# databendlabs/databend

Measured on AMD Instinct MI355X. Metric: rows/s TPC-H Q1 hash-agg, higher is better.
Workload: dtype i64/i128 decimal

## Files before the change

### databend_amd/csrc/gbk_api.h

```cpp

extern "C" {

int32_t dbhip_group_hash(const dbhip_col* cols, int32_t ncols, int64_t n, uint64_t* out_hashes,
                         void* stream) {
  DBHIP_REQUIRE(cols && ncols >= 1 && ncols <= GB_MAX_KEYS, "dbhip_group_hash: bad column list");
  if (n == 0) return DBHIP_OK;
  DBHIP_REQUIRE(out_hashes, "dbhip_group_hash: NULL out");
  HashCols hc;
  hc.n = ncols;
  for (int k = 0; k < ncols; ++k) {
    if (!key_type_ok(cols[k].type)) {
      set_error("dbhip_group_hash: unsupported type %d", cols[k].type);
      return DBHIP_ERR_INVALID;
    }
    hc.c[k] = to_gbcol(cols[k]);
  }
  hipStream_t s = resolve_stream(stream);
  unsigned long long* bad = (unsigned long long*)scratch(8, 2, s);
  if (!bad) return DBHIP_ERR_HIP;
  DBHIP_CHECK(hipMemsetAsync(bad, 0, 8, s));
  hipLaunchKernelGGL(group_hash_kernel, dim3(grid_for(ceil_div(n, 4), 256, 1024)), dim3(256), 0, s, hc, n, out_hashes, bad);
  DBHIP_LAUNCH_CHECK();
  return DBHIP_OK;
}
// ... 287 lines not shown
  g->rows_seen = 0;
}
static int32_t ensure_xcur(dbhip_groupby* g);
constexpr int GB_CTRL_XSTATUS = 12;
static int32_t blocks_queued(dbhip_groupby* g, const uint64_t* blocks, int32_t n_blocks, int64_t max_rows, int32_t skip, bool replace,
                             const char* who, hipStream_t s) {
  const int W = g->L.W;
  const int64_t stride = (max_rows + 1) * W;
  const int64_t ub = (int64_t)(n_blocks - (skip >= 0 && skip < n_blocks ? 1 : 0)) * max_rows;
  if (ub == 0) return DBHIP_OK;
  int32_t rc;
  if ((rc = ensure_xcur(g))) return rc;
  if ((rc = ensure((void**)&g->rows_in, &g->rows_in_cap, (size_t)ub * W * 8))) return rc;
  if ((rc = ensure((void**)&g->gid, &g->gid_cap, (size_t)ub * 4))) return rc;
  if ((rc = ensure((void**)&g->retry, &g->retry_cap, (size_t)ub * 4))) return rc;
  uint64_t* host = pinned_words(0);
  if (!host) return DBHIP_ERR_HIP;
  uint64_t* xst = g->ctrl + GB_CTRL_XSTATUS;
  if (replace)
    hipLaunchKernelGGL(gb_reset_unless_off_kernel, dim3(grid_for(g->cap, 256, 256)), dim3(256), 0, s, blocks, stride, n_blocks, max_rows, g->slot_hash, g->cap, g->ctrl);
  hipLaunchKernelGGL(gb_compact_blocks_kernel, dim3(n_blocks), dim3(256), 0, s, blocks, stride, W, skip, g->rows_in, xst, n_blocks, max_rows, replace ? 1 : 0);
  DBHIP_LAUNCH_CHECK();
  if ((rc = merge_rows_unpinned(g, g->rows_in, ub, s, xst, xst + 1, 2))) return rc;
  DBHIP_CHECK(hipMemcpyAsync(host, g->ctrl, (GB_CTRL_XSTATUS + 3) * sizeof(uint64_t), hipMemcpyDeviceToHost, s));
  DBHIP_CHECK(hipStreamSynchronize(s));
  if (host[GB_CTRL_XSTATUS + 1]) {
    set_error("%s: block %d overflowed max_rows=%lld (exchange the rows with dbhip_groupby_flush_partitioned / flush_serialized + "
              "merge_serialized instead)", who, (int)host[GB_CTRL_XSTATUS + 2] - 1, (long long)max_rows);
    return DBHIP_ERR_CAPACITY;
  }
  if (replace) reset_host_state(g);
  g->count_host = (int64_t)host[0];
  if (host[3] & 2) {
    set_error("groupby: a string key longer than 12 bytes was met; keep the CPU operator for this block");
    return DBHIP_ERR_UNSUPPORTED;
  }
  if (host[1]) {
    set_error("groupby: collision chain filled the table during retry; create the table with a larger capacity");
    return DBHIP_ERR_CAPACITY;
  }
  return host[GB_CTRL_XSTATUS] ? pin_string_states(g, s) : DBHIP_OK;
}

int32_t dbhip_groupby_merge_blocks(dbhip_groupby* g, const void* blocks_dev, int32_t n_blocks, int64_t max_rows,
                                   int32_t skip_block, void* stream) {
  GB_DRAIN(g, resolve_stream(stream));
  DBHIP_REQUIRE(g && blocks_dev && n_blocks >= 1 && n_blocks <= 4096 && max_rows >= 1, "dbhip_groupby_merge_blocks: bad argument");
  if (int32_t rl = refuse_long_strings(g, "dbhip_groupby_merge_blocks")) return rl;
// ... 329 lines not shown
```

### databend_amd/csrc/gbk_merge_lds.h

```cpp

namespace {

int32_t ensure(void** p, size_t* cap, size_t bytes) {
  if (*cap >= bytes) return DBHIP_OK;
  if (*p) {
    int32_t rc = dbhip_free(*p);
    if (rc) return rc;
    *p = nullptr; *cap = 0;
  }
  size_t want = bytes + (bytes >> 3) + 256;
  int32_t rc = dbhip_alloc(want, p);
  if (rc) { *p = nullptr; return rc; }
  *cap = want;
  return DBHIP_OK;
}

int32_t alloc_table(dbhip_groupby* g, int64_t cap, hipStream_t s) {
  uint64_t* nh = nullptr;
  uint64_t* nr = nullptr;
  int32_t rc = dbhip_alloc((size_t)cap * 8, (void**)&nh);
  if (rc == DBHIP_OK) rc = dbhip_alloc((size_t)cap * g->L.W * 8, (void**)&nr);
  hipError_t e = rc == DBHIP_OK ? hipMemsetAsync(nh, 0, (size_t)cap * 8, s) : hipSuccess;
  if (rc != DBHIP_OK || e != hipSuccess) {
    if (nh) (void)dbhip_free(nh);
// ... 131 lines not shown
  DBHIP_CHECK(hipMemsetAsync(&g->ctrl[8], 0, 8, s));
  hipLaunchKernelGGL(gb_pin_strings_kernel, dim3(grid), dim3(256), 0, s, g->L, g->slot_hash, g->rows, g->cap, (uint64_t)g->arena,
                     (uint64_t)g->arena + g->arena_cap, 4, na, (int64_t)0, g->ctrl, acc);
  DBHIP_LAUNCH_CHECK();
  DBHIP_CHECK(hipStreamSynchronize(s));
  trace("groupby: string arena compacted, %llu bytes in use -> %llu live (capacity %zu -> %zu)",
        (unsigned long long)two[1], (unsigned long long)two[0], g->arena_cap, want);
  (void)dbhip_free(g->arena);
  g->arena = na;
  g->arena_cap = want;
  return DBHIP_OK;
}
int32_t reserve_arena_for_chunk(dbhip_groupby* g, hipStream_t s) {
  uint64_t lb = 0;
  DBHIP_CHECK(hipMemcpyAsync(&lb, &g->ctrl[9], 8, hipMemcpyDeviceToHost, s));
  DBHIP_CHECK(hipStreamSynchronize(s));
  if (lb == 0) return DBHIP_OK;
  g->has_long = 1;
  return reserve_arena(g, lb, s);
}
bool layout_has_strings(const GbLayout& L) { return L.str_w1_mask != 0; }
bool layout_has_wide_minmax(const GbLayout& L);

int32_t merge_rows_unpinned(dbhip_groupby* g, const uint64_t* rows_in, int64_t n, hipStream_t s, const uint64_t* n_dev, const uint64_t* abort_dev,
                            int deferred = 0);
int32_t merge_rows(dbhip_groupby* g, const uint64_t* rows_in, int64_t n, hipStream_t s,
                   const uint64_t* n_dev = nullptr, const uint64_t* abort_dev = nullptr) {
  int32_t rc = merge_rows_unpinned(g, rows_in, n, s, n_dev, abort_dev);
  if (rc == DBHIP_OK && n > 0) rc = pin_string_states(g, s);
  return rc;
}
int32_t merge_rows_unpinned(dbhip_groupby* g, const uint64_t* rows_in, int64_t n, hipStream_t s,
                            const uint64_t* n_dev, const uint64_t* abort_dev, int deferred) {
  if (n == 0) return DBHIP_OK;
  if (n > 0xFFFFFFF0LL) {
    set_error("groupby: more than 2^32 rows in one call");
    return DBHIP_ERR_INVALID;
  }
  int32_t rc;
  if ((rc = ensure((void**)&g->gid, &g->gid_cap, (size_t)n * 4))) return rc;
  if ((rc = ensure((void**)&g->retry, &g->retry_cap, (size_t)n * 4))) return rc;
  const int grid = grid_for(n, 256);
  uint64_t* host_ctrl = pinned_words(0);
  if (!host_ctrl) return DBHIP_ERR_HIP;
  const uint64_t* cur_rows = rows_in;
  int64_t cur_n = n;
  const DevCount dc{n_dev, abort_dev};
  if ((deferred || (g->count_host + n) * 135 <= g->cap * 100) && n <= 256) {
    hipLaunchKernelGGL(gb_merge_small_kernel, dim3(1), dim3(256), 0, s, g->L, cur_rows, cur_n, g->slot_hash, g->rows, g->cap, g->hash_mask, g->gid,
                       g->retry, g->ctrl, dc, g->arena);
    DBHIP_LAUNCH_CHECK();
    if (deferred) return DBHIP_OK;
    DBHIP_CHECK(hipMemcpyAsync(host_ctrl, g->ctrl, 5 * sizeof(uint64_t), hipMemcpyDeviceToHost, s));
    DBHIP_CHECK(hipStreamSynchronize(s));
    g->count_host = (int64_t)host_ctrl[0];
    if (host_ctrl[3] & 2) {
      set_error("groupby: a string key longer than 12 bytes was met; keep the CPU operator for this block");
      return DBHIP_ERR_UNSUPPORTED;
    }
    if (host_ctrl[1]) {
      set_error("groupby: collision chain filled the table during retry; create the table with a larger capacity");
      return DBHIP_ERR_CAPACITY;
    }
    return DBHIP_OK;
  }
  if (deferred || (g->count_host + n) * 135 <= g->cap * 100) {
    DBHIP_CHECK(hipMemsetAsync(&g->ctrl[1], 0, 16, s));
    hipLaunchKernelGGL(gb_probe_kernel, dim3(grid), dim3(256), 0, s, g->L, cur_rows, cur_n, g->slot_hash, g->rows, g->cap,
                       g->hash_mask, g->gid, g->ctrl, dc, g->arena);
    if (deferred == 1 || (!deferred && g->count_host > 0 && g->count_host <= 32 && n <= 65536) || n <= 2048 || layout_has_wide_minmax(g->L))
      hipLaunchKernelGGL(gb_accum_lowcard_kernel, dim3(deferred == 1 && grid > 16 ? 16 : grid), dim3(256), 0, s, g->L, cur_rows, cur_n, g->rows, g->gid, g->retry,
// ... 323 lines not shown
```

### databend_amd/csrc/gbk_rows.h

```cpp

namespace {

struct HashCols {
  GbCol c[GB_MAX_KEYS];
  int n;
};

__global__ __launch_bounds__(256) void group_hash_kernel(HashCols hc, int64_t n, uint64_t* out,
                                                         unsigned long long* bad) {
  constexpr int U = 4;
  const int64_t T = (int64_t)gridDim.x * blockDim.x;
  const int64_t t = (int64_t)blockIdx.x * blockDim.x + threadIdx.x;
  for (int64_t base = 0; base < n; base += U * T) {
    int64_t row[U];
    bool in[U];
    uint64_t h[U];
#pragma unroll
    for (int u = 0; u < U; ++u) {
      row[u] = base + u * T + t;
      in[u] = row[u] < n;
      if (!in[u]) row[u] = n - 1;
      h[u] = 0;
    }
    for (int k = 0; k < hc.n; ++k) {
// ... 315 lines not shown

__device__ __forceinline__ uint64_t wave_min_u64(uint64_t v) {
#pragma unroll
  for (int off = 32; off >= 1; off >>= 1) {
    uint64_t o = __shfl_xor(v, off, 64);
    v = o < v ? o : v;
  }
  return v;
}
__device__ __forceinline__ uint64_t wave_max_u64(uint64_t v) {
#pragma unroll
  for (int off = 32; off >= 1; off >>= 1) {
    uint64_t o = __shfl_xor(v, off, 64);
    v = o > v ? o : v;
  }
  return v;
}
__device__ __forceinline__ double wave_sum_f64(double v) {
#pragma unroll
  for (int off = 32; off >= 1; off >>= 1) v += __shfl_xor(v, off, 64);
  return v;
}

__device__ __forceinline__ void gb_accum_lowcard_body(const GbLayout& L, const uint64_t* rows_in,
                                                      int64_t n, uint64_t* rows,
                                                      const uint32_t* gid, uint32_t* retry,
                                                      uint64_t* ctrl, const uint8_t* arena) {
  const int64_t n_pad = (n + 63) & ~63LL;
  for (int64_t i = (int64_t)blockIdx.x * blockDim.x + threadIdx.x; i < n_pad;
       i += (int64_t)gridDim.x * blockDim.x) {
    bool active = i < n;
    const uint64_t* r = rows_in + (active ? i : 0) * L.W;
    uint32_t pos = active ? gid[i] : GB_INVALID_SLOT;
    if (active) {
      const uint64_t* d = rows + (uint64_t)pos * L.W;
      if (!keys_equal(L, r, d, arena)) {
        unsigned long long k = atomicAdd((unsigned long long*)&ctrl[2], 1ULL);
        retry[k] = (uint32_t)i;
        active = false;
      }
    }
    uint64_t todo = __ballot(active);
    while (todo) {
      int leader = __ffsll((long long)todo) - 1;
      uint32_t lpos = __shfl(pos, leader, 64);
      bool mine = active && pos == lpos;
// ... 95 lines not shown
  }
}
__global__ void gb_retry_kernel(GbLayout L, const uint64_t* rows_in, uint64_t* slot_hash, uint64_t* rows,
                                int64_t cap, uint64_t hash_mask, const uint32_t* gid,
                                const uint32_t* retry, uint64_t* ctrl, uint8_t* arena) {
  if (threadIdx.x != 0 || blockIdx.x != 0) return;
  gb_retry_body(L, rows_in, slot_hash, rows, cap, hash_mask, gid, retry, ctrl, arena);
}

__global__ __launch_bounds__(256) void gb_merge_small_kernel(GbLayout L, const uint64_t* rows_in, int64_t n, uint64_t* slot_hash, uint64_t* rows,
                                                             int64_t cap, uint64_t hash_mask, uint32_t* gid, uint32_t* retry, uint64_t* ctrl,
                                                             DevCount dc, uint8_t* arena) {
  n = dev_rows(dc, n);
  if (threadIdx.x < 2) ctrl[1 + threadIdx.x] = 0;
  __threadfence();
  __syncthreads();
  gb_probe_body(L, rows_in, n, slot_hash, rows, cap, hash_mask, gid, ctrl, arena);
  __threadfence();
  __syncthreads();
  gb_accum_lowcard_body(L, rows_in, n, rows, gid, retry, ctrl, arena);
  __threadfence();
  __syncthreads();
  if (threadIdx.x == 0) gb_retry_body(L, rows_in, slot_hash, rows, cap, hash_mask, gid, retry, ctrl, arena);
}

__global__ __launch_bounds__(256) void gb_rehash_kernel(GbLayout L, const uint64_t* old_hash,
                                                        const uint64_t* old_rows, int64_t old_cap,
                                                        uint64_t* new_hash, uint64_t* new_rows,
                                                        int64_t new_cap, uint64_t hash_mask) {
  const uint64_t cmask = (uint64_t)new_cap - 1;
  for (int64_t s = (int64_t)blockIdx.x * blockDim.x + threadIdx.x; s < old_cap;
       s += (int64_t)gridDim.x * blockDim.x) {
    uint64_t hw = old_hash[s];
    if (hw == 0) continue;
    const uint64_t* r = old_rows + s * L.W;
    uint64_t pos = home_slot(probe_word(r[L.hash_word], hash_mask), new_cap);
    while (true) {
      unsigned long long old = atomicCAS((unsigned long long*)&new_hash[pos], 0ULL, (unsigned long long)hw);
      if (old == 0) break;
      pos = (pos + 1) & cmask;
    }
    uint64_t* d = new_rows + pos * L.W;
    for (int k = 0; k < L.W; ++k) d[k] = r[k];
  }
}

// ... 493 lines not shown
```

### databend_amd/csrc/k_fagg.hip

```cpp
#include "fagg_device.h"
#include "runtime.h"

#include <dirent.h>
#include <dlfcn.h>
#include <errno.h>
#include <sys/stat.h>
#include <fcntl.h>
#include <signal.h>
#include <spawn.h>
#include <sys/wait.h>
#include <unistd.h>

#include <atomic>
#include <chrono>
#include <deque>
#include <map>
#include <mutex>
#include <string>

#include <stdlib.h>
#include <string.h>
#include <time.h>

using namespace dbhip;

int32_t dbhip_groupby_merge_rows_dev_internal(dbhip_groupby* g, const uint64_t* rows, int64_t n_max, const uint64_t* n_dev,
                                              const uint64_t* abort_dev, hipStream_t s);
int32_t dbhip_groupby_merge_rows_internal(dbhip_groupby* g, const uint64_t* rows, int64_t n, hipStream_t s);
int64_t dbhip_groupby_capacity_internal(dbhip_groupby* g);
int32_t dbhip_groupby_reserve_merge_internal(dbhip_groupby* g, int64_t n);
int64_t dbhip_groupby_count_internal(dbhip_groupby* g);
const GbLayout* dbhip_groupby_layout_internal(dbhip_groupby* g);
int32_t dbhip_groupby_merge_rows_deferred_internal(dbhip_groupby* g, const uint64_t* rows, int64_t n_max, const uint64_t* n_dev,
                                                   const uint64_t* abort_dev, hipStream_t s);
int32_t dbhip_groupby_ensure_room_internal(dbhip_groupby* g, int64_t extra, hipStream_t s);
uint64_t* dbhip_groupby_ctrl_internal(dbhip_groupby* g);
void dbhip_groupby_set_count_internal(dbhip_groupby* g, int64_t count);
void** dbhip_groupby_pipe_slot_internal(dbhip_groupby* g);

namespace {

#include "build/jit_embed.inc"

struct JitOut {
  std::string s;
  void num(long long v) { s += std::to_string(v); s += ","; }
  void u64(uint64_t v) { char b[40]; snprintf(b, sizeof(b), "0x%llxULL,", (unsigned long long)v); s += b; }
  void null() { s += "nullptr,"; }
  void open() { s += "{"; }
  void close() { s += "},"; }
};

void jit_ins(JitOut& o, const ExIns& I) {
// ... 879 lines not shown
    pp->bound = true; pp->stream = s;
    return fa_pipe_enqueue(g, pp, P, s);
  }
  FaArgs A;
  memset(&A, 0, sizeof(A));
  bool general = false, may_raise = false;
  int nwords = 0;
  int32_t rc = fa_build_args(L, keys, prog, A, &general, &nwords, &may_raise);
  if (rc) return rc;
  A.filter_bits = filter_bitmap; A.filter_off = filter_bit_offset; A.n = n;
  A.has_filter = filter_bitmap != nullptr;
  const size_t lds = (size_t)(A.P.n_slots > 6 ? A.P.n_slots : 6) * FA_ROWS * 256 * 8;
  if (lds > 60 * 1024) {
    set_error("dbhip_groupby_add_block_program: %d live LDS slots exceed the register file; split the expression", A.P.n_slots);
    return DBHIP_ERR_UNSUPPORTED;
  }
  const int64_t nchunks = ceil_div(n, 64 * FA_ROWS);
  const int grid = (int)(ceil_div(nchunks, 4) < 512 ? ceil_div(nchunks, 4) : 512);
  if (FaPipe* pp = (FaPipe*)*dbhip_groupby_pipe_slot_internal(g); pp && !t_prepare_only) {
    int64_t committed = 0;
    if ((rc = fa_pipe_checkpoint(g, pp, &committed, true))) return rc;
  }
  const size_t rows_bytes = (size_t)grid * FA_MAX_SLOTS * L.W * 8;
  uint8_t* ws = (uint8_t*)scratch(rows_bytes + 64, 6, s);
  if (!ws) return DBHIP_ERR_HIP;
  uint64_t* ctrl = (uint64_t*)ws;
  A.ctrl = ctrl;
  A.partial_rows = (uint64_t*)(ws + 64);
  A.P.err_words = nullptr;
  A.P.err_count = (unsigned long long*)&ctrl[2];
  uint64_t* host_ctrl = pinned_words(1);
  if (!host_ctrl) return DBHIP_ERR_HIP;
  host_ctrl[0] = host_ctrl[1] = host_ctrl[2] = 0;
  const int64_t n_max = (int64_t)grid * FA_MAX_SLOTS;
  const bool chained = (dbhip_groupby_count_internal(g) + n_max) * 135 <= dbhip_groupby_capacity_internal(g) * 100;
  if ((rc = dbhip_groupby_reserve_merge_internal(g, n_max))) return rc;
  if (t_prepare_only) {
    (void)jit_kernel(A, dbhip_groupby_count_internal(g) > 4 ? 8 : 4, general, nwords, JIT_COMPILE);
    if (FaPipe* pq = (FaPipe*)*dbhip_groupby_pipe_slot_internal(g); pq && pq->on)
      (void)jit_kernel(A, dbhip_groupby_count_internal(g) > 4 ? 8 : 4, general, nwords, JIT_COMPILE, nullptr, true);
    return DBHIP_OK;
  }
  for (int variant = dbhip_groupby_count_internal(g) > 4 ? 1 : 0; variant < 2; ++variant) {
    DBHIP_CHECK(hipMemsetAsync(ctrl, 0, 64, s));
    kernel_timer_start(s);
    if ((rc = fa_launch(A, variant == 0 ? 4 : 8, general, nwords, grid, lds, s))) return rc;
    kernel_timer_stop(s);
    DBHIP_LAUNCH_CHECK();
    DBHIP_CHECK(hipMemcpyAsync(host_ctrl, ctrl, 24, hipMemcpyDeviceToHost, s));
    if (chained && !may_raise) {
      rc = dbhip_groupby_merge_rows_dev_internal(g, A.partial_rows, n_max, &ctrl[0], &ctrl[1], s);
      if (rc) return rc;
      if (!(host_ctrl[1] & 3)) return DBHIP_OK;
    } else {
      DBHIP_CHECK(hipStreamSynchronize(s));
    }
    if (!(host_ctrl[1] & 1)) break;
  }
  if (host_ctrl[1] & 2) {
    set_error("dbhip_groupby_add_block_program: a group key string is longer than 12 bytes");
    return DBHIP_ERR_UNSUPPORTED;
  }
  if (host_ctrl[1] & 1) {
    set_error("dbhip_groupby_add_block_program: more than %d distinct groups inside one workgroup; use the operator-at-a-time path", FA_MAX_SLOTS);
    return DBHIP_ERR_CAPACITY;
  }
  if (host_ctrl[2]) {
    set_error("dbhip_groupby_add_block_program: %llu row error(s) in the fused maps (Decimal overflow / divided by zero); "
              "evaluate the maps with dbhip_expr_eval to get the rows", (unsigned long long)host_ctrl[2]);
    return DBHIP_ERR_ROW_ERRORS;
  }
  return dbhip_groupby_merge_rows_internal(g, A.partial_rows, (int64_t)host_ctrl[0], s);
}

int32_t dbhip_groupby_set_pipelined(dbhip_groupby* g, int32_t on, void* stream) {
  DBHIP_REQUIRE(g, "dbhip_groupby_set_pipelined: NULL argument");
  void** slot = dbhip_groupby_pipe_slot_internal(g);
// ... 203 lines not shown
```

### databend_amd/csrc/k_groupby.hip

```cpp
#include <mutex>
#include "gb_device.h"
#include "runtime.h"

#include <math.h>
#include <stdlib.h>
#include <string.h>

#include <new>
#include <vector>

using namespace dbhip;

#define GB_INVALID_SLOT 0xFFFFFFFFu

struct dbhip_groupby {
  int64_t hint_groups;
  GbLayout L;
  int64_t cap;
  uint64_t* slot_hash;
  uint64_t* rows;
  uint64_t* ctrl;
  uint64_t hash_mask;
  int64_t count_host;
  uint64_t* rows_in; size_t rows_in_cap;
// ... 10 lines not shown
  int part_direct;
  int part_adapt;
  int part_validate, part_validated;
  int64_t rows_seen;
  uint32_t* part_meta; size_t part_meta_cap;
  uint32_t* spill_idx; size_t spill_idx_cap;
  uint64_t* spill_rows; size_t spill_rows_cap;
  uint8_t* arena; size_t arena_cap;
  int has_long;
  uint64_t* xcur;
  int xcur_dirty;
  int fagg_disabled;
  int gbc_off;
  int gbc_active;
  int gbc_lcap;
  int gbc_nodirect;
  int gbc_part_lcap_max;
  uint32_t gbc_part_cap;
  uint64_t* gbc_spill; size_t gbc_spill_cap;
  uint64_t arena_pinned, arena_live;
  int gbc_skip;
  uint32_t* gbc_split; size_t gbc_split_cap;
  void* fa_pipe;
};

int32_t dbhip_fagg_pipe_drain_internal(dbhip_groupby* g, void* pipe, hipStream_t s);
void dbhip_fagg_pipe_destroy_internal(void* pipe);
int32_t dbhip_fagg_pipe_reset_internal(void* pipe, hipStream_t s);
struct GbCols;
int32_t dbhip_fagg_pipe_add_columns_internal(dbhip_groupby* g, void* pipe, const GbCols& C, int64_t n, hipStream_t s);
#define GB_DRAIN(g, s)                                                                   \
  do {                                                                                   \
    if ((g) && (g)->fa_pipe) {                                                           \
      const int32_t _rc = dbhip_fagg_pipe_drain_internal((g), (g)->fa_pipe, (s));        \
      if (_rc) return _rc;                                                               \
    }                                                                                    \
  } while (0)

#include "gbk_rows.h"
int32_t dbhip_groupby_build_layout_internal(const int32_t* key_types, const uint8_t* key_nullable, int nkeys, const dbhip_agg_desc* aggs,
                                            int naggs, GbLayout* L) {
  return build_layout(key_types, key_nullable, nkeys, aggs, naggs, L);
}
#include "gbk_merge_lds.h"
int32_t dbhip_fagg_add_columns_internal(dbhip_groupby* g, const GbCols& C, int64_t row0, int64_t n, bool may_compile, hipStream_t s);
bool dbhip_fagg_last_refusal_is_pending_internal();
#include "gbk_partitioned.h"

int32_t dbhip_groupby_merge_rows_internal(dbhip_groupby* g, const uint64_t* rows, int64_t n, hipStream_t s) {
  return merge_rows(g, rows, n, s);
}
int32_t dbhip_groupby_merge_rows_dev_internal(dbhip_groupby* g, const uint64_t* rows, int64_t n_max, const uint64_t* n_dev,
                                              const uint64_t* abort_dev, hipStream_t s) {
  return merge_rows(g, rows, n_max, s, n_dev, abort_dev);
}
int32_t dbhip_groupby_reserve_merge_internal(dbhip_groupby* g, int64_t n) {
  int32_t rc;
  if ((rc = ensure((void**)&g->gid, &g->gid_cap, (size_t)n * 4))) return rc;
  return ensure((void**)&g->retry, &g->retry_cap, (size_t)n * 4);
}
int32_t dbhip_groupby_merge_rows_deferred_internal(dbhip_groupby* g, const uint64_t* rows, int64_t n_max, const uint64_t* n_dev,
                                                   const uint64_t* abort_dev, hipStream_t s) {
  return merge_rows_unpinned(g, rows, n_max, s, n_dev, abort_dev, 1);
}
int32_t dbhip_groupby_ensure_room_internal(dbhip_groupby* g, int64_t extra, hipStream_t s) {
  uint64_t cnt = 0;
  DBHIP_CHECK(hipMemcpyAsync(&cnt, &g->ctrl[0], 8, hipMemcpyDeviceToHost, s));
  DBHIP_CHECK(hipStreamSynchronize(s));
  g->count_host = (int64_t)cnt;
  while ((g->count_host + extra) * 135 > g->cap * 100) {
    const int32_t rc = grow(g, s);
    if (rc) return rc;
  }
  return DBHIP_OK;
}
uint64_t* dbhip_groupby_ctrl_internal(dbhip_groupby* g) { return g->ctrl; }
void dbhip_groupby_set_count_internal(dbhip_groupby* g, int64_t count) { g->count_host = count; }
void** dbhip_groupby_pipe_slot_internal(dbhip_groupby* g) { return &g->fa_pipe; }
// ... 6 lines not shown
```

### databend_amd/csrc/k_q1.hip

```cpp
#include "gb_device.h"
#include "runtime.h"

#include <stdlib.h>
#include <string.h>

using namespace dbhip;

int32_t dbhip_groupby_merge_rows_internal(dbhip_groupby* g, const uint64_t* rows, int64_t n, hipStream_t s);
int32_t dbhip_groupby_merge_rows_dev_internal(dbhip_groupby* g, const uint64_t* rows, int64_t n_max, const uint64_t* n_dev,
                                              const uint64_t* abort_dev, hipStream_t s);
int64_t dbhip_groupby_capacity_internal(dbhip_groupby* g);
int64_t dbhip_groupby_count_internal(dbhip_groupby* g);
const GbLayout* dbhip_groupby_layout_internal(dbhip_groupby* g);

namespace {

constexpr int MAX_SLOTS = 8;
constexpr int Q1_W = 15;

struct alignas(16) U4 {
  uint32_t x, y, z, w;
};
struct alignas(16) L2 {
  int64_t a, b;
};
struct alignas(8) I2 {
  int32_t a, b;
};

typedef uint32_t q1_u32x4 __attribute__((ext_vector_type(4)));
typedef uint32_t q1_u32x2 __attribute__((ext_vector_type(2)));
__device__ __forceinline__ U4 ld_u4(const U4* p) { return __builtin_bit_cast(U4, __builtin_nontemporal_load((const q1_u32x4*)p)); }
__device__ __forceinline__ L2 ld_l2(const int64_t* p) { return __builtin_bit_cast(L2, __builtin_nontemporal_load((const q1_u32x4*)p)); }
__device__ __forceinline__ I2 ld_i2(const int32_t* p) { return __builtin_bit_cast(I2, __builtin_nontemporal_load((const q1_u32x2*)p)); }

// ... 264 lines not shown

int32_t dbhip_q1_fused(dbhip_groupby* g, const int64_t* l_quantity, const int64_t* l_extendedprice,
                       const int64_t* l_discount, const int64_t* l_tax, const void* l_returnflag_views,
                       const void* l_linestatus_views, const int32_t* l_shipdate, int32_t shipdate_cutoff,
                       int64_t n, void* stream) {
  DBHIP_REQUIRE(g, "dbhip_q1_fused: NULL table");
  const GbLayout* L = dbhip_groupby_layout_internal(g);
  bool layout_ok = L->nkeys == 2 && L->naggs == 6 && L->W == Q1_W && L->key_type[0] == DBHIP_T_STRING &&
                   L->key_type[1] == DBHIP_T_STRING && L->agg_off[0] == 5 && L->agg_off[2] == 7 &&
                   L->agg_off[5] == 14 && L->agg_words[2] == 3 && L->agg_words[3] == 3;
  DBHIP_REQUIRE(layout_ok, "dbhip_q1_fused: table was not created by dbhip_q1_create_groupby");
  if (n == 0) return DBHIP_OK;
  DBHIP_REQUIRE(l_quantity && l_extendedprice && l_discount && l_tax && l_returnflag_views &&
                    l_linestatus_views && l_shipdate,
                "dbhip_q1_fused: NULL column");
  uintptr_t al = (uintptr_t)l_quantity | (uintptr_t)l_extendedprice | (uintptr_t)l_discount |
                 (uintptr_t)l_tax | (uintptr_t)l_returnflag_views | (uintptr_t)l_linestatus_views;
  DBHIP_REQUIRE((al & 15) == 0 && ((uintptr_t)l_shipdate & 7) == 0,
                "dbhip_q1_fused: columns must be 16-byte aligned (shipdate 8-byte)");
  hipStream_t s = resolve_stream(stream);
  const int64_t ntiles = ceil_div(n, 128);
  const int grid = (int)(ceil_div(ntiles, 4) < 512 ? ceil_div(ntiles, 4) : 512);
  size_t rows_bytes = (size_t)grid * MAX_SLOTS * Q1_W * 8;
  uint8_t* ws = (uint8_t*)scratch(rows_bytes + 64, 4, s);
  if (!ws) return DBHIP_ERR_HIP;
  uint64_t* ctrl = (uint64_t*)ws;
  uint64_t* partial = (uint64_t*)(ws + 64);
  Q1Args A;
  A.qty = l_quantity; A.price = l_extendedprice; A.disc = l_discount; A.tax = l_tax;
  A.rf = (const U4*)l_returnflag_views; A.ls = (const U4*)l_linestatus_views;
  A.shipdate = l_shipdate; A.cutoff = shipdate_cutoff; A.n = n;
  A.partial_rows = partial; A.ctrl = ctrl;
  uint64_t* host_ctrl = pinned_words(1);
  if (!host_ctrl) return DBHIP_ERR_HIP;
  host_ctrl[0] = host_ctrl[1] = 0;
  const int64_t n_max4 = (int64_t)grid * 4, n_max8 = (int64_t)grid * MAX_SLOTS;
  const bool chained = (dbhip_groupby_count_internal(g) + n_max8) * 135 <= dbhip_groupby_capacity_internal(g) * 100;
  for (int variant = 0; variant < 2; ++variant) {
    DBHIP_CHECK(hipMemsetAsync(ctrl, 0, 64, s));
    kernel_timer_start(s);
    if (variant == 0) hipLaunchKernelGGL(q1_fused_kernel, dim3(grid), dim3(256), 0, s, A);
    else hipLaunchKernelGGL(q1_fused_kernel_8slots, dim3(grid), dim3(256), 0, s, A);
    kernel_timer_stop(s);
    DBHIP_LAUNCH_CHECK();
    DBHIP_CHECK(hipMemcpyAsync(host_ctrl, ctrl, 16, hipMemcpyDeviceToHost, s));
    if (chained) {
      int32_t rc = dbhip_groupby_merge_rows_dev_internal(g, partial, variant == 0 ? n_max4 : n_max8, &ctrl[0], &ctrl[1], s);
      if (rc) return rc;
      if (!(host_ctrl[1] & 3)) return DBHIP_OK;
    } else {
      DBHIP_CHECK(hipStreamSynchronize(s));
    }
    if (!(host_ctrl[1] & 1)) break;
  }
  if (host_ctrl[1] & 2) {
    set_error("dbhip_q1_fused: a group key string is longer than 12 bytes; use the operator-at-a-time path");
    return DBHIP_ERR_UNSUPPORTED;
  }
  if (host_ctrl[1] & 1) {
    set_error("dbhip_q1_fused: more than %d distinct groups inside one workgroup; use the operator-at-a-time path", MAX_SLOTS);
    return DBHIP_ERR_CAPACITY;
  }
  return dbhip_groupby_merge_rows_internal(g, partial, (int64_t)host_ctrl[0], s);
}

}
```

### databend_amd/csrc/runtime.h

```cpp
#pragma once
#include <hip/hip_runtime.h>
#include <stdint.h>
#include <stdio.h>
#include <stdlib.h>

#include "../../include/dbhip.h"

namespace dbhip {

void set_error(const char* fmt, ...);
hipStream_t resolve_stream(void* stream);
int32_t hip_fail(hipError_t e, const char* what);

void* scratch(size_t bytes, int slot, hipStream_t stream);
void release_stream_scratch(hipStream_t stream);

bool cancel_requested(hipStream_t stream);

uint64_t* pinned_words(int slot);

void kernel_timer_start(hipStream_t s);
void kernel_timer_stop(hipStream_t s);


void trace(const char* fmt, ...) __attribute__((format(printf, 1, 2)));

inline int64_t ceil_div(int64_t a, int64_t b) { return (a + b - 1) / b; }

inline int grid_for(int64_t n_items_per_thread_units, int block, int cap = 2048) {
  int64_t need = ceil_div(n_items_per_thread_units, block);
  if (need < 1) need = 1;
  if (need > cap) need = cap;
  return (int)need;
}

inline int type_size(int32_t t) {
  switch (t) {
    case DBHIP_T_I8: case DBHIP_T_U8: return 1;
    case DBHIP_T_I16: case DBHIP_T_U16: return 2;
    case DBHIP_T_I32: case DBHIP_T_U32: case DBHIP_T_F32: case DBHIP_T_DATE: return 4;
    case DBHIP_T_I64: case DBHIP_T_U64: case DBHIP_T_F64: case DBHIP_T_TIMESTAMP:
    case DBHIP_T_DEC64: return 8;
// ... 37 lines not shown
```

### databend_amd/csrc/runtime.hip

```cpp
#include "runtime.h"

#include <stdarg.h>
#include <string.h>

#include <stdlib.h>

#include <sys/syscall.h>
#include <unistd.h>

#include <atomic>
#include <map>
#include <mutex>
#include <new>
#include <unordered_map>
#include <vector>

namespace dbhip {

static thread_local char g_err[512] = "";
static hipStream_t g_stream = nullptr;
static int g_device = -1;
static std::mutex g_mu;

struct Scratch {
  void* p = nullptr;
  size_t cap = 0;
};
struct StreamScratch {
  Scratch slot[25];
  uint64_t last_use = 0;
};
constexpr size_t SCRATCH_STREAMS_PER_THREAD = 8;
struct ScratchKey {
  uint64_t tid;
  hipStream_t stream;
  bool operator<(const ScratchKey& o) const { return tid != o.tid ? tid < o.tid : (uintptr_t)stream < (uintptr_t)o.stream; }
};
static std::mutex g_scratch_mu;
static std::map<ScratchKey, StreamScratch>* g_scratch = nullptr;
static std::atomic<uint64_t> g_scratch_clock{0};
static std::atomic<uint64_t> g_next_tid{1};

static void free_entry(StreamScratch& e) {
  for (Scratch& s : e.slot) {
    if (s.p) (void)hipFree(s.p);
    s.p = nullptr;
    s.cap = 0;
  }
}
static void release_scratch_entries(uint64_t tid, hipStream_t stream, bool any_stream) {
  std::lock_guard<std::mutex> lk(g_scratch_mu);
  if (!g_scratch) return;
  for (auto it = g_scratch->begin(); it != g_scratch->end();) {
    const bool hit = (tid == 0 || it->first.tid == tid) && (any_stream || it->first.stream == stream);
    if (hit) { free_entry(it->second); it = g_scratch->erase(it); } else ++it;
  }
}
struct ThreadScratchOwner {
  uint64_t tid = g_next_tid.fetch_add(1);
  bool is_main = false;
  ThreadScratchOwner() { is_main = (long)getpid() == (long)syscall(SYS_gettid); }
  ~ThreadScratchOwner() {
    if (is_main) return;
// ... 13 lines not shown
void trace(const char* fmt, ...) {
  static const bool on = getenv("DBHIP_TRACE") != nullptr;
  if (!on) return;
  va_list ap;
  va_start(ap, fmt);
  flockfile(stderr);
  fputs("[dbhip] ", stderr);
  vfprintf(stderr, fmt, ap);
  fputc('\n', stderr);
  funlockfile(stderr);
  va_end(ap);
}

int32_t hip_fail(hipError_t e, const char* what) {
  set_error("HIP error %d (%s) in %s", (int)e, hipGetErrorString(e), what);
  return DBHIP_ERR_HIP;
}

hipStream_t resolve_stream(void* stream) {
  if (stream) return (hipStream_t)stream;
  return g_stream;
}

void* scratch(size_t bytes, int slot, hipStream_t stream) {
  const uint64_t tid = t_scratch_owner.tid;
  Scratch* sp = nullptr;
  StreamScratch evicted;
  bool have_evicted = false;
  {
    std::lock_guard<std::mutex> lk(g_scratch_mu);
    if (!g_scratch) g_scratch = new (std::nothrow) std::map<ScratchKey, StreamScratch>();
    if (!g_scratch) { set_error("scratch: out of host memory"); return nullptr; }
    const ScratchKey key{tid, stream};
    auto it = g_scratch->find(key);
    if (it == g_scratch->end()) {
      size_t mine = 0;
      auto lru = g_scratch->end();
      for (auto j = g_scratch->lower_bound(ScratchKey{tid, nullptr}); j != g_scratch->end() && j->first.tid == tid; ++j) {
        ++mine;
        if (lru == g_scratch->end() || j->second.last_use < lru->second.last_use) lru = j;
      }
      if (mine >= SCRATCH_STREAMS_PER_THREAD && lru != g_scratch->end()) {
        evicted = lru->second;
        have_evicted = true;
        g_scratch->erase(lru);
      }
      it = g_scratch->emplace(key, StreamScratch()).first;
    }
    it->second.last_use = g_scratch_clock.fetch_add(1) + 1;
    sp = &it->second.slot[slot];
  }
  if (have_evicted) {
    (void)hipDeviceSynchronize();
    free_entry(evicted);
  }
  Scratch& s = *sp;
  if (s.cap < bytes) {
    if (s.p) {
      (void)hipStreamSynchronize(stream);
      (void)hipFree(s.p);
    }
    size_t cap = bytes + (bytes >> 2) + 4096;
    if (hipMalloc(&s.p, cap) != hipSuccess) {
      s.p = nullptr;
      s.cap = 0;
      set_error("scratch allocation of %zu bytes failed", cap);
      return nullptr;
    }
    s.cap = cap;
  }
  return s.p;
}

void release_stream_scratch(hipStream_t stream) { release_scratch_entries(0, stream, false); }

static std::atomic<int> g_cancel_any{0};
static std::mutex g_cancel_mu;
static std::unordered_map<hipStream_t, int>* g_cancelled = nullptr;
bool cancel_requested(hipStream_t stream) {
  if (g_cancel_any.load(std::memory_order_relaxed) == 0) return false;
  std::lock_guard<std::mutex> lk(g_cancel_mu);
  return g_cancelled && g_cancelled->count(stream) != 0;
}
static void set_cancel(hipStream_t stream, bool on) {
  std::lock_guard<std::mutex> lk(g_cancel_mu);
  if (!g_cancelled) g_cancelled = new (std::nothrow) std::unordered_map<hipStream_t, int>();
  if (!g_cancelled) return;
  if (on) (*g_cancelled)[stream] = 1; else g_cancelled->erase(stream);
  g_cancel_any.store((int)g_cancelled->size(), std::memory_order_relaxed);
}

static thread_local uint64_t* g_pinned = nullptr;
uint64_t* pinned_words(int slot) {
  if (!g_pinned) {
    void* p = nullptr;
    if (hipHostMalloc(&p, 8 * 64 * sizeof(uint64_t), hipHostMallocDefault) != hipSuccess) return nullptr;
    g_pinned = (uint64_t*)p;
  }
  return g_pinned + (slot & 7) * 64;
}

static thread_local hipEvent_t g_t0 = nullptr, g_t1 = nullptr;
static thread_local bool g_timed = false;

void kernel_timer_start(hipStream_t s) {
  if (!g_t0) {
    if (hipEventCreate(&g_t0) != hipSuccess || hipEventCreate(&g_t1) != hipSuccess) { g_t0 = g_t1 = nullptr; return; }
  }
  (void)hipEventRecord(g_t0, s);
  g_timed = false;
}

void kernel_timer_stop(hipStream_t s) {
  if (!g_t1) return;
  (void)hipEventRecord(g_t1, s);
  g_timed = true;
}

}

using namespace dbhip;

// ... 228 lines not shown
```

Baseline: 91.34 billion.

## Fold small merges into one kernel writing status to mapped host memory

Adds a single-block fold-merge kernel that probes, merges partial rows through an LDS staging table, retries, and writes control status straight into mapped pinned host memory tagged with a sequence number. The Q1 and fused-agg paths use it in place of the separate memcpy plus merge launches. The ctrl memset is skipped when the previous fold kernel already zeroed it, which is tracked through a new scratch generation counter. The aim is to cut launch, memset and device-to-host copy overhead per call, at the cost of a serial 1024-thread merge and more complex status handling.

```diff
diff --git a/databend_amd/csrc/gbk_api.h b/databend_amd/csrc/gbk_api.h
--- a/databend_amd/csrc/gbk_api.h
+++ b/databend_amd/csrc/gbk_api.h
@@ -333,8 +333,15 @@
   hipLaunchKernelGGL(gb_compact_blocks_kernel, dim3(n_blocks), dim3(256), 0, s, blocks, stride, W, skip, g->rows_in, xst, n_blocks, max_rows, replace ? 1 : 0);
   DBHIP_LAUNCH_CHECK();
   if ((rc = merge_rows_unpinned(g, g->rows_in, ub, s, xst, xst + 1, 2))) return rc;
-  DBHIP_CHECK(hipMemcpyAsync(host, g->ctrl, (GB_CTRL_XSTATUS + 3) * sizeof(uint64_t), hipMemcpyDeviceToHost, s));
-  DBHIP_CHECK(hipStreamSynchronize(s));
+  if (g->fold_seq) {
+    DBHIP_CHECK(hipStreamSynchronize(s));
+    const uint64_t* st = fold_status(g);
+    if (!st) return DBHIP_ERR_HIP;
+    for (int i = 0; i < GB_CTRL_XSTATUS + 3; ++i) host[i] = st[8 + i];
+  } else {
+    DBHIP_CHECK(hipMemcpyAsync(host, g->ctrl, (GB_CTRL_XSTATUS + 3) * sizeof(uint64_t), hipMemcpyDeviceToHost, s));
+    DBHIP_CHECK(hipStreamSynchronize(s));
+  }
   if (host[GB_CTRL_XSTATUS + 1]) {
     set_error("%s: block %d overflowed max_rows=%lld (exchange the rows with dbhip_groupby_flush_partitioned / flush_serialized + "
               "merge_serialized instead)", who, (int)host[GB_CTRL_XSTATUS + 2] - 1, (long long)max_rows);
diff --git a/databend_amd/csrc/gbk_merge_lds.h b/databend_amd/csrc/gbk_merge_lds.h
--- a/databend_amd/csrc/gbk_merge_lds.h
+++ b/databend_amd/csrc/gbk_merge_lds.h
@@ -177,6 +177,44 @@
 bool layout_has_strings(const GbLayout& L) { return L.str_w1_mask != 0; }
 bool layout_has_wide_minmax(const GbLayout& L);
 
+int32_t merge_outcome(dbhip_groupby* g, const uint64_t* host_ctrl) {
+  g->count_host = (int64_t)host_ctrl[0];
+  if (host_ctrl[3] & 2) {
+    set_error("groupby: a string key longer than 12 bytes was met; keep the CPU operator for this block");
+    return DBHIP_ERR_UNSUPPORTED;
+  }
+  if (host_ctrl[1]) {
+    set_error("groupby: collision chain filled the table during retry; create the table with a larger capacity");
+    return DBHIP_ERR_CAPACITY;
+  }
+  return DBHIP_OK;
+}
+static std::atomic<uint64_t> g_fold_seq{0};
+const uint64_t* fold_status(dbhip_groupby* g) {
+  uint64_t* dev = nullptr;
+  const uint64_t* st = mapped_status(&dev);
+  if (!st || __atomic_load_n(&st[24], __ATOMIC_ACQUIRE) != g->fold_seq) {
+    set_error("groupby: the merge kernel left no status (sequence %llu expected)", (unsigned long long)g->fold_seq);
+    return nullptr;
+  }
+  return st;
+}
+int32_t fold_merge(dbhip_groupby* g, const uint64_t* rows_in, int64_t n, hipStream_t s, const DevCount& dc, uint64_t* pctrl, bool drain,
+                   const uint64_t** status_out) {
+  uint64_t* status_dev = nullptr;
+  if (!mapped_status(&status_dev)) { set_error("groupby: no mapped host memory for the merge status"); return DBHIP_ERR_HIP; }
+  g->fold_seq = g_fold_seq.fetch_add(1) + 1;
+  hipLaunchKernelGGL(gb_fold_merge_kernel, dim3(1), dim3(GB_FOLD_THREADS), 0, s, g->L, rows_in, n, g->slot_hash, g->rows, g->cap, g->hash_mask,
+                     g->gid, g->retry, g->ctrl, dc, g->arena, pctrl, status_dev, g->fold_seq);
+  DBHIP_LAUNCH_CHECK();
+  if (!drain) return DBHIP_OK;
+  DBHIP_CHECK(hipStreamSynchronize(s));
+  const uint64_t* st = fold_status(g);
+  if (!st) return DBHIP_ERR_HIP;
+  if (status_out) *status_out = st;
+  return merge_outcome(g, st + 8);
+}
+
 int32_t merge_rows_unpinned(dbhip_groupby* g, const uint64_t* rows_in, int64_t n, hipStream_t s, const uint64_t* n_dev, const uint64_t* abort_dev,
                             int deferred = 0);
 int32_t merge_rows(dbhip_groupby* g, const uint64_t* rows_in, int64_t n, hipStream_t s,
@@ -201,7 +239,11 @@
   const uint64_t* cur_rows = rows_in;
   int64_t cur_n = n;
   const DevCount dc{n_dev, abort_dev};
-  if ((deferred || (g->count_host + n) * 135 <= g->cap * 100) && n <= 256) {
+  const bool no_growth = deferred || (g->count_host + n) * 135 <= g->cap * 100;
+  g->fold_seq = 0;
+  if (no_growth && n <= GB_FOLD_MAX_ROWS && (deferred == 0 || (deferred == 2 && g->count_host <= 32)))
+    return fold_merge(g, cur_rows, cur_n, s, dc, nullptr, deferred == 0, nullptr);
+  if (no_growth && n <= 256) {
     hipLaunchKernelGGL(gb_merge_small_kernel, dim3(1), dim3(256), 0, s, g->L, cur_rows, cur_n, g->slot_hash, g->rows, g->cap, g->hash_mask, g->gid,
                        g->retry, g->ctrl, dc, g->arena);
     DBHIP_LAUNCH_CHECK();
diff --git a/databend_amd/csrc/gbk_rows.h b/databend_amd/csrc/gbk_rows.h
--- a/databend_amd/csrc/gbk_rows.h
+++ b/databend_amd/csrc/gbk_rows.h
@@ -361,6 +361,42 @@
   return v;
 }
 
+struct GbStage {
+  uint64_t* rows;
+  uint32_t* tag;
+  uint32_t* used;
+  int K;
+};
+__device__ __forceinline__ bool gb_fold_covers(const GbLayout& L, int a) { return !gb_minmax_wide(L, a) && !gb_sum256(L, a); }
+__device__ __forceinline__ uint64_t* gb_stage_row(const GbStage& S, const GbLayout& L, uint32_t pos) {
+  const uint32_t kmask = (uint32_t)S.K - 1;
+  uint32_t e = ((pos * 0x9E3779B1u) >> 16) & kmask;
+  const int steps = *(volatile uint32_t*)S.used >= (uint32_t)S.K ? (S.K < 4 ? S.K : 4) : S.K;
+  for (int step = 0; step < steps; ++step) {
+    const uint32_t cur = atomicCAS(&S.tag[e], 0u, pos + 1);
+    if (cur == 0) atomicAdd(S.used, 1u);
+    if (cur == 0 || cur == pos + 1) return S.rows + (size_t)e * L.W;
+    e = (e + 1) & kmask;
+  }
+  return nullptr;
+}
+__device__ __forceinline__ void gb_fold_body(const GbLayout& L, const uint64_t* rows_in, int64_t n, uint64_t* rows, const uint32_t* gid,
+                                             uint32_t* retry, uint64_t* ctrl, const uint8_t* arena, const GbStage& S) {
+  for (int64_t i = threadIdx.x; i < n; i += blockDim.x) {
+    const uint64_t* r = rows_in + i * L.W;
+    const uint32_t pos = gid[i];
+    if (pos == GB_INVALID_SLOT) continue;
+    uint64_t* d = rows + (uint64_t)pos * L.W;
+    if (!keys_equal(L, r, d, arena)) {
+      unsigned long long k = atomicAdd((unsigned long long*)&ctrl[2], 1ULL);
+      retry[k] = (uint32_t)i;
+      continue;
+    }
+    uint64_t* st = S.K ? gb_stage_row(S, L, pos) : nullptr;
+    for (int a = 0; a < L.naggs; ++a) gb_atomic_merge(L, a, ((st && gb_fold_covers(L, a)) ? st : d) + L.agg_off[a], r + L.agg_off[a]);
+  }
+}
+
 __device__ __forceinline__ void gb_accum_lowcard_body(const GbLayout& L, const uint64_t* rows_in,
                                                       int64_t n, uint64_t* rows,
                                                       const uint32_t* gid, uint32_t* retry,
@@ -502,6 +538,54 @@
   __threadfence();
   __syncthreads();
   if (threadIdx.x == 0) gb_retry_body(L, rows_in, slot_hash, rows, cap, hash_mask, gid, retry, ctrl, arena);
+}
+
+constexpr int GB_FOLD_THREADS = 1024;
+constexpr int GB_FOLD_LDS_WORDS = 4096;
+constexpr int GB_FOLD_KMAX = 64;
+constexpr int64_t GB_FOLD_MAX_ROWS = 4096;
+__global__ __launch_bounds__(GB_FOLD_THREADS) void gb_fold_merge_kernel(GbLayout L, const uint64_t* rows_in, int64_t n, uint64_t* slot_hash,
+                                                                        uint64_t* rows, int64_t cap, uint64_t hash_mask, uint32_t* gid,
+                                                                        uint32_t* retry, uint64_t* ctrl, DevCount dc, uint8_t* arena,
+                                                                        uint64_t* pctrl, uint64_t* status, uint64_t seq) {
+  __shared__ uint64_t st_rows[GB_FOLD_LDS_WORDS];
+  __shared__ uint32_t st_tag[GB_FOLD_KMAX];
+  __shared__ uint32_t st_used;
+  GbStage S{st_rows, st_tag, &st_used, GB_FOLD_KMAX};
+  while (S.K && S.K * L.W > GB_FOLD_LDS_WORDS) S.K >>= 1;
+  n = dev_rows(dc, n);
+  if (pctrl && pctrl[2]) n = 0;
+  const int tid = threadIdx.x;
+  if (tid < 2) ctrl[1 + tid] = 0;
+  if (tid < GB_FOLD_KMAX) st_tag[tid] = 0;
+  if (tid == 0) st_used = 0;
+  for (int x = tid; x < S.K * L.naggs; x += GB_FOLD_THREADS) gb_state_identity(L, x % L.naggs, st_rows + (size_t)(x / L.naggs) * L.W + L.agg_off[x % L.naggs]);
+  __threadfence();
+  __syncthreads();
+  gb_probe_body(L, rows_in, n, slot_hash, rows, cap, hash_mask, gid, ctrl, arena);
+  __threadfence();
+  __syncthreads();
+  gb_fold_body(L, rows_in, n, rows, gid, retry, ctrl, arena, S);
+  __threadfence();
+  __syncthreads();
+  for (int x = tid; x < S.K * L.naggs; x += GB_FOLD_THREADS) {
+    const int e = x / L.naggs, a = x % L.naggs;
+    const uint32_t tag = st_tag[e];
+    if (tag == 0 || !gb_fold_covers(L, a)) continue;
+    gb_atomic_merge(L, a, rows + (uint64_t)(tag - 1) * L.W + L.agg_off[a], st_rows + (size_t)e * L.W + L.agg_off[a]);
+  }
+  __threadfence();
+  __syncthreads();
+  if (tid == 0) gb_retry_body(L, rows_in, slot_hash, rows, cap, hash_mask, gid, retry, ctrl, arena);
+  __threadfence();
+  if (tid < 24) {
+    uint64_t* src = tid < 8 ? (pctrl ? pctrl + tid : nullptr) : ctrl + (tid - 8);
+    const uint64_t v = src ? __hip_atomic_load(src, __ATOMIC_RELAXED, __HIP_MEMORY_SCOPE_AGENT) : 0;
+    __hip_atomic_store(&status[tid], v, __ATOMIC_RELAXED, __HIP_MEMORY_SCOPE_SYSTEM);
+    if (tid < 8 && pctrl) pctrl[tid] = 0;
+  }
+  __threadfence_system();
+  if (tid == 0) __hip_atomic_store(&status[24], seq, __ATOMIC_RELEASE, __HIP_MEMORY_SCOPE_SYSTEM);
 }
 
 __global__ __launch_bounds__(256) void gb_rehash_kernel(GbLayout L, const uint64_t* old_hash,
diff --git a/databend_amd/csrc/k_fagg.hip b/databend_amd/csrc/k_fagg.hip
--- a/databend_amd/csrc/k_fagg.hip
+++ b/databend_amd/csrc/k_fagg.hip
@@ -29,6 +29,7 @@
 int32_t dbhip_groupby_merge_rows_internal(dbhip_groupby* g, const uint64_t* rows, int64_t n, hipStream_t s);
 int64_t dbhip_groupby_capacity_internal(dbhip_groupby* g);
 int32_t dbhip_groupby_reserve_merge_internal(dbhip_groupby* g, int64_t n);
+int32_t dbhip_groupby_fold_merge_internal(dbhip_groupby* g, const uint64_t* rows, int64_t n_max, uint64_t* pctrl, hipStream_t s, uint64_t* out);
 int64_t dbhip_groupby_count_internal(dbhip_groupby* g);
 const GbLayout* dbhip_groupby_layout_internal(dbhip_groupby* g);
 int32_t dbhip_groupby_merge_rows_deferred_internal(dbhip_groupby* g, const uint64_t* rows, int64_t n_max, const uint64_t* n_dev,
@@ -954,7 +955,8 @@
     if ((rc = fa_pipe_checkpoint(g, pp, &committed, true))) return rc;
   }
   const size_t rows_bytes = (size_t)grid * FA_MAX_SLOTS * L.W * 8;
-  uint8_t* ws = (uint8_t*)scratch(rows_bytes + 64, 6, s);
+  uint64_t ws_gen = 0;
+  uint8_t* ws = (uint8_t*)scratch(rows_bytes + 64, 6, s, &ws_gen);
   if (!ws) return DBHIP_ERR_HIP;
   uint64_t* ctrl = (uint64_t*)ws;
   A.ctrl = ctrl;
@@ -973,18 +975,24 @@
       (void)jit_kernel(A, dbhip_groupby_count_internal(g) > 4 ? 8 : 4, general, nwords, JIT_COMPILE, nullptr, true);
     return DBHIP_OK;
   }
+  static thread_local struct { const void* p; uint64_t gen; } t_zeroed = {nullptr, 0};
   for (int variant = dbhip_groupby_count_internal(g) > 4 ? 1 : 0; variant < 2; ++variant) {
-    DBHIP_CHECK(hipMemsetAsync(ctrl, 0, 64, s));
+    const bool zeroed = t_zeroed.p == ws && t_zeroed.gen == ws_gen;
+    t_zeroed.p = nullptr;
+    if (!zeroed) DBHIP_CHECK(hipMemsetAsync(ctrl, 0, 64, s));
     kernel_timer_start(s);
     if ((rc = fa_launch(A, variant == 0 ? 4 : 8, general, nwords, grid, lds, s))) return rc;
     kernel_timer_stop(s);
     DBHIP_LAUNCH_CHECK();
-    DBHIP_CHECK(hipMemcpyAsync(host_ctrl, ctrl, 24, hipMemcpyDeviceToHost, s));
-    if (chained && !may_raise) {
-      rc = dbhip_groupby_merge_rows_dev_internal(g, A.partial_rows, n_max, &ctrl[0], &ctrl[1], s);
+    if (chained) {
+      uint64_t st[4];
+      rc = dbhip_groupby_fold_merge_internal(g, A.partial_rows, n_max, ctrl, s, st);
+      if (st[3]) { t_zeroed.p = ws; t_zeroed.gen = ws_gen; }
       if (rc) return rc;
-      if (!(host_ctrl[1] & 3)) return DBHIP_OK;
+      host_ctrl[0] = st[0]; host_ctrl[1] = st[1]; host_ctrl[2] = st[2];
+      if (!(host_ctrl[1] & 3) && !host_ctrl[2]) return DBHIP_OK;
     } else {
+      DBHIP_CHECK(hipMemcpyAsync(host_ctrl, ctrl, 24, hipMemcpyDeviceToHost, s));
       DBHIP_CHECK(hipStreamSynchronize(s));
     }
     if (!(host_ctrl[1] & 1)) break;
diff --git a/databend_amd/csrc/k_groupby.hip b/databend_amd/csrc/k_groupby.hip
--- a/databend_amd/csrc/k_groupby.hip
+++ b/databend_amd/csrc/k_groupby.hip
@@ -1,3 +1,4 @@
+#include <atomic>
 #include <mutex>
 #include "gb_device.h"
 #include "runtime.h"
@@ -56,6 +57,7 @@
   int gbc_skip;
   uint32_t* gbc_split; size_t gbc_split_cap;
   void* fa_pipe;
+  uint64_t fold_seq;
 };
 
 int32_t dbhip_fagg_pipe_drain_internal(dbhip_groupby* g, void* pipe, hipStream_t s);
@@ -88,6 +90,14 @@
                                               const uint64_t* abort_dev, hipStream_t s) {
   return merge_rows(g, rows, n_max, s, n_dev, abort_dev);
 }
+int32_t dbhip_groupby_fold_merge_internal(dbhip_groupby* g, const uint64_t* rows, int64_t n_max, uint64_t* pctrl, hipStream_t s, uint64_t* out) {
+  out[0] = out[1] = out[2] = out[3] = 0;
+  const uint64_t* st = nullptr;
+  int32_t rc = fold_merge(g, rows, n_max, s, DevCount{&pctrl[0], &pctrl[1]}, pctrl, true, &st);
+  if (st) { out[0] = st[0]; out[1] = st[1]; out[2] = st[2]; out[3] = 1; }
+  if (rc == DBHIP_OK && out[0] > 0 && !(out[1] & 3) && !out[2]) rc = pin_string_states(g, s);
+  return rc;
+}
 int32_t dbhip_groupby_reserve_merge_internal(dbhip_groupby* g, int64_t n) {
   int32_t rc;
   if ((rc = ensure((void**)&g->gid, &g->gid_cap, (size_t)n * 4))) return rc;
diff --git a/databend_amd/csrc/k_q1.hip b/databend_amd/csrc/k_q1.hip
--- a/databend_amd/csrc/k_q1.hip
+++ b/databend_amd/csrc/k_q1.hip
@@ -11,6 +11,8 @@
                                               const uint64_t* abort_dev, hipStream_t s);
 int64_t dbhip_groupby_capacity_internal(dbhip_groupby* g);
 int64_t dbhip_groupby_count_internal(dbhip_groupby* g);
+int32_t dbhip_groupby_reserve_merge_internal(dbhip_groupby* g, int64_t n);
+int32_t dbhip_groupby_fold_merge_internal(dbhip_groupby* g, const uint64_t* rows, int64_t n_max, uint64_t* pctrl, hipStream_t s, uint64_t* out);
 const GbLayout* dbhip_groupby_layout_internal(dbhip_groupby* g);
 
 namespace {
@@ -321,7 +323,8 @@
   const int64_t ntiles = ceil_div(n, 128);
   const int grid = (int)(ceil_div(ntiles, 4) < 512 ? ceil_div(ntiles, 4) : 512);
   size_t rows_bytes = (size_t)grid * MAX_SLOTS * Q1_W * 8;
-  uint8_t* ws = (uint8_t*)scratch(rows_bytes + 64, 4, s);
+  uint64_t ws_gen = 0;
+  uint8_t* ws = (uint8_t*)scratch(rows_bytes + 64, 4, s, &ws_gen);
   if (!ws) return DBHIP_ERR_HIP;
   uint64_t* ctrl = (uint64_t*)ws;
   uint64_t* partial = (uint64_t*)(ws + 64);
@@ -335,19 +338,29 @@
   host_ctrl[0] = host_ctrl[1] = 0;
   const int64_t n_max4 = (int64_t)grid * 4, n_max8 = (int64_t)grid * MAX_SLOTS;
   const bool chained = (dbhip_groupby_count_internal(g) + n_max8) * 135 <= dbhip_groupby_capacity_internal(g) * 100;
+  if (chained) {
+    int32_t rc = dbhip_groupby_reserve_merge_internal(g, n_max8);
+    if (rc) return rc;
+  }
+  static thread_local struct { const void* p; uint64_t gen; } t_zeroed = {nullptr, 0};
   for (int variant = 0; variant < 2; ++variant) {
-    DBHIP_CHECK(hipMemsetAsync(ctrl, 0, 64, s));
+    const bool zeroed = t_zeroed.p == ws && t_zeroed.gen == ws_gen;
+    t_zeroed.p = nullptr;
+    if (!zeroed) DBHIP_CHECK(hipMemsetAsync(ctrl, 0, 64, s));
     kernel_timer_start(s);
     if (variant == 0) hipLaunchKernelGGL(q1_fused_kernel, dim3(grid), dim3(256), 0, s, A);
     else hipLaunchKernelGGL(q1_fused_kernel_8slots, dim3(grid), dim3(256), 0, s, A);
     kernel_timer_stop(s);
     DBHIP_LAUNCH_CHECK();
-    DBHIP_CHECK(hipMemcpyAsync(host_ctrl, ctrl, 16, hipMemcpyDeviceToHost, s));
     if (chained) {
-      int32_t rc = dbhip_groupby_merge_rows_dev_internal(g, partial, variant == 0 ? n_max4 : n_max8, &ctrl[0], &ctrl[1], s);
+      uint64_t st[4];
+      int32_t rc = dbhip_groupby_fold_merge_internal(g, partial, variant == 0 ? n_max4 : n_max8, ctrl, s, st);
+      if (st[3]) { t_zeroed.p = ws; t_zeroed.gen = ws_gen; }
       if (rc) return rc;
+      host_ctrl[0] = st[0]; host_ctrl[1] = st[1];
       if (!(host_ctrl[1] & 3)) return DBHIP_OK;
     } else {
+      DBHIP_CHECK(hipMemcpyAsync(host_ctrl, ctrl, 16, hipMemcpyDeviceToHost, s));
       DBHIP_CHECK(hipStreamSynchronize(s));
     }
     if (!(host_ctrl[1] & 1)) break;
diff --git a/databend_amd/csrc/runtime.h b/databend_amd/csrc/runtime.h
--- a/databend_amd/csrc/runtime.h
+++ b/databend_amd/csrc/runtime.h
@@ -12,12 +12,13 @@
 hipStream_t resolve_stream(void* stream);
 int32_t hip_fail(hipError_t e, const char* what);
 
-void* scratch(size_t bytes, int slot, hipStream_t stream);
+void* scratch(size_t bytes, int slot, hipStream_t stream, uint64_t* gen_out = nullptr);
 void release_stream_scratch(hipStream_t stream);
 
 bool cancel_requested(hipStream_t stream);
 
 uint64_t* pinned_words(int slot);
+uint64_t* mapped_status(uint64_t** dev_out);
 
 void kernel_timer_start(hipStream_t s);
 void kernel_timer_stop(hipStream_t s);
diff --git a/databend_amd/csrc/runtime.hip b/databend_amd/csrc/runtime.hip
--- a/databend_amd/csrc/runtime.hip
+++ b/databend_amd/csrc/runtime.hip
@@ -25,6 +25,7 @@
 struct Scratch {
   void* p = nullptr;
   size_t cap = 0;
+  uint64_t gen = 0;
 };
 struct StreamScratch {
   Scratch slot[25];
@@ -39,6 +40,7 @@
 static std::mutex g_scratch_mu;
 static std::map<ScratchKey, StreamScratch>* g_scratch = nullptr;
 static std::atomic<uint64_t> g_scratch_clock{0};
+static std::atomic<uint64_t> g_scratch_gen{0};
 static std::atomic<uint64_t> g_next_tid{1};
 
 static void free_entry(StreamScratch& e) {
@@ -98,7 +100,7 @@
   return g_stream;
 }
 
-void* scratch(size_t bytes, int slot, hipStream_t stream) {
+void* scratch(size_t bytes, int slot, hipStream_t stream, uint64_t* gen_out) {
   const uint64_t tid = t_scratch_owner.tid;
   Scratch* sp = nullptr;
   StreamScratch evicted;
@@ -144,7 +146,9 @@
       return nullptr;
     }
     s.cap = cap;
-  }
+    s.gen = g_scratch_gen.fetch_add(1) + 1;
+  }
+  if (gen_out) *gen_out = s.gen;
   return s.p;
 }
 
@@ -174,6 +178,22 @@
     g_pinned = (uint64_t*)p;
   }
   return g_pinned + (slot & 7) * 64;
+}
+
+static thread_local uint64_t* g_status = nullptr;
+static thread_local uint64_t* g_status_dev = nullptr;
+uint64_t* mapped_status(uint64_t** dev_out) {
+  if (!g_status) {
+    void* p = nullptr;
+    void* d = nullptr;
+    if (hipHostMalloc(&p, 64 * sizeof(uint64_t), hipHostMallocMapped) != hipSuccess) return nullptr;
+    if (hipHostGetDevicePointer(&d, p, 0) != hipSuccess) { (void)hipHostFree(p); return nullptr; }
+    memset(p, 0, 64 * sizeof(uint64_t));
+    g_status = (uint64_t*)p;
+    g_status_dev = (uint64_t*)d;
+  }
+  *dev_out = g_status_dev;
+  return g_status;
 }
 
 static thread_local hipEvent_t g_t0 = nullptr, g_t1 = nullptr;
```

Result: no change. 91.24 billion (-0.1%).
